# tud-amr/mpc_planner

Hardware: AMD Instinct MI355X
Metric: MPC solves/s (Jackal N=20, 8 obs) (higher is better)
Workload: dtype f64

## Files before the change

mpc_planner_amd/csrc/tmpc_kernels.hpp:

```cpp
#pragma once
#include <hip/hip_runtime.h>
#include <math.h>
#include <stdint.h>
#include <stdio.h>
#include <stdlib.h>
#include <string.h>
#include <string>
#include <type_traits>
#include <vector>

#include "../../include/tmpc_hip.h"
#include "tmpc_stage.hpp"

namespace tmpc {

constexpr int NT = 64;

static __constant__ int c_pi[NP28] = {0, 1, 1, 2, 2, 2, 3, 3, 3, 3, 4, 4, 4, 4, 4, 5, 5, 5, 5, 5, 5, 6, 6, 6, 6, 6, 6, 6};
static __constant__ int c_pj[NP28] = {0, 0, 1, 0, 1, 2, 0, 1, 2, 3, 0, 1, 2, 3, 4, 0, 1, 2, 3, 4, 5, 0, 1, 2, 3, 4, 5, 6};

enum { ST_KEEP_ITERATE = 1, ST_KEEP_MULTIPLIERS = 2, ST_STORE = 4, ST_COMPLETE = 8 };
struct StateIO {
    double *z;
    double *pi;
    double *lamh;
    int *stopped;
    int flags;
    double *ws;
    int *ticket;
    const int *slot;
    int *valid;
    const int *share;
};
__device__ __forceinline__ int param_base_of(const StateIO &io, int b) { return io.share ? io.share[b] : b; }
__device__ __forceinline__ int slot_of(const StateIO &io, int b) { return io.slot ? io.slot[b] : b; }
__device__ __forceinline__ int slot_flags(const StateIO &io, int b)
{
    if (!(io.flags & (ST_KEEP_ITERATE | ST_KEEP_MULTIPLIERS))) return io.flags;
    return io.valid[slot_of(io, b)] ? io.flags : (io.flags & ~(ST_KEEP_ITERATE | ST_KEEP_MULTIPLIERS));
}

struct Lds {
    double *z, *pi, *W, *g, *BA, *b, *D, *beta;
    double *t, *lam, *invt, *qt;
    double *v, *pq, *Hh, *rg, *gh, *rb, *dv, *dpi, *pr, *y, *rdiag, *scr;
    double *dyn8;
    double *lamh;
    int nh, NG, GB, XB, nrows;
    double *tab;
    int n_pair, dstride;
    double *scan;
};

constexpr int BAC_1 = 8, BAC_SDT = 9, BAC_SH = 10, BAC_0 = 11, BAC_DT = 12, BA_NCONST = 20;
constexpr int BAR_S = 5, BAR_PSI = 12, BAR_V = 13;
constexpr int BAP_X = 16, BAP_Y = 15, BAP_S = 7;
constexpr int BAT_A = 3, BAT_W = 6, BAT_XY = 7, BAT_PSI = 16, BAT_V = 9, BAT_S = 17;
constexpr unsigned ba_pack(int a, int w, int x, int y, int p, int v, int s_)
{
    return (unsigned)a | (unsigned)w << 4 | (unsigned)x << 8 | (unsigned)y << 12 | (unsigned)p << 16 | (unsigned)v << 20 | (unsigned)s_ << 24;
}
__device__ __forceinline__ constexpr unsigned ba_rowcode(int m)
{
    return m == 0 ? ba_pack(0, 2, BAC_1, BAC_0, 4, 6, BAC_0)
         : m == 1 ? ba_pack(1, 3, BAC_0, BAC_1, 5, 7, BAC_0)
         : m == 2 ? ba_pack(BAC_0, BAC_DT, BAC_0, BAC_0, BAC_1, BAC_0, BAC_0)
         : m == 3 ? ba_pack(BAC_DT, BAC_0, BAC_0, BAC_0, BAC_0, BAC_1, BAC_0)
                  : ba_pack(BAC_SH, BAC_0, BAC_0, BAC_0, BAC_0, BAC_SDT, BAC_1);
}
__device__ __forceinline__ int ba_off(int N, int k, int m, int j)
{
    const unsigned rc = m == 0 ? ba_rowcode(0) : m == 1 ? ba_rowcode(1) : m == 2 ? ba_rowcode(2) : m == 3 ? ba_rowcode(3) : ba_rowcode(4);
    const int code = (int)((rc >> (4 * j)) & 15u);
    return code < 8 ? k * 8 + code : N * 8 + code - 8;
}
__device__ __forceinline__ void ba_tab_init(double *tab, const Dims &d, int tid)
{
    if (tid < BA_NCONST) {
        const double dt = d.dt, sdt = d.sdt, sh = d.shdt2;
        const double c[BA_NCONST] = {1.0, sdt, sh, 0.0, dt,   sh, dt, 0.0, 0.0, 0.0, 1.0, sdt,   0.0, dt, dt, 0.0, 1.0, 0.0, 0.0, 1.0};
        double val = 0.0;
#pragma unroll
        for (int i = 0; i < BA_NCONST; i++) if (i == tid) val = c[i];
        tab[d.N * 8 + tid] = val;
    }
}
__host__ __device__ inline int ws_doubles(int N, bool two_wave = false)
{
    return (N + 1) * NV + (N + 1) * NX + (N + 1) * NP28 + (N + 1) * NV + (N + 1) * NX + (two_wave ? N * NP28 : 0);
}


__host__ __device__ inline int lds_doubles(int N, int nh)
{
    const int nrows = N * nh + 4 * N + 10 * (N - 1);
    int n = 0;
    n += (N + 1) * NV + (N + 1) * NX + (N + 1) * NP28 + (N + 1) * NV + N * NX * NV + N * NX + N * nh * 3 + N * nh;
    n += 4 * nrows;
    n += (N + 1) * NV + (N + 1) * NX + (N + 1) * NP28 + 2 * (N + 1) * NV + N * NX + (N + 1) * NV + (N + 1) * NX +
         (N + 1) * NX + N * NU + N * NU + 64 + N * 8;
    return n;
}

__host__ __device__ inline bool split_rows_for(int N, int nh)
{
    return 2 * N * nh <= (N + 1) * (NV + NX + NP28 + NV + NV) + N * NX && 12 * (N + 1) >= 12 * N;
}

__device__ __forceinline__ Lds carve(double *s, const Dims &d)
{
    Lds L;
    const int N = d.N;
    L.nh = d.n_up + d.M;
    L.NG = N * L.nh; L.GB = L.NG; L.XB = L.NG + 4 * N; L.nrows = L.XB + 10 * (N - 1);
    auto take = [&](int n) { double *p = s; s += n; return p; };
    L.z = take((N + 1) * NV); L.pi = take((N + 1) * NX); L.W = take((N + 1) * NP28); L.g = take((N + 1) * NV);
    L.BA = take(N * NX * NV); L.b = take(N * NX); L.D = take(N * L.nh * 3); L.beta = take(N * L.nh);
    L.t = take(L.nrows); L.lam = take(L.nrows); L.invt = take(L.nrows); L.qt = take(L.nrows);
    L.v = take((N + 1) * NV); L.pq = take((N + 1) * NX); L.Hh = take((N + 1) * NP28);
    L.rg = take((N + 1) * NV); L.gh = take((N + 1) * NV); L.rb = take(N * NX); L.dv = take((N + 1) * NV);
    L.dpi = take((N + 1) * NX); L.pr = take((N + 1) * NX); L.y = take(N * NU); L.rdiag = take(N * NU);
    L.scr = take(64); L.dyn8 = take(N * 8);
    L.lamh = nullptr;
    return L;
}

__device__ __forceinline__ int trajectory_of_block(int blk, int B)
{
    (void)B;
    return blk;
}

template <int CTRL, int ROW_MASK>
__device__ __forceinline__ double dpp_move(double x, double identity)
{
    union { double d; int i[2]; } u, o;
    u.d = x; o.d = identity;
    o.i[0] = __builtin_amdgcn_update_dpp(o.i[0], u.i[0], CTRL, ROW_MASK, 0xf, false);
    o.i[1] = __builtin_amdgcn_update_dpp(o.i[1], u.i[1], CTRL, ROW_MASK, 0xf, false);
    return o.d;
}
template <int CTRL>
__device__ __forceinline__ double dpp_shift_zero(double x)
{
    union { double d; int i[2]; } u, o;
    u.d = x;
    o.i[0] = __builtin_amdgcn_mov_dpp(u.i[0], CTRL, 0xf, 0xf, true);
    o.i[1] = __builtin_amdgcn_mov_dpp(u.i[1], CTRL, 0xf, 0xf, true);
    return o.d;
}
template <typename Op>
__device__ __forceinline__ double wave_reduce(double x, double identity, Op op)
{
    x = op(x, dpp_move<0x111, 0xf>(x, identity));
    x = op(x, dpp_move<0x112, 0xf>(x, identity));
    x = op(x, dpp_move<0x114, 0xf>(x, identity));
    x = op(x, dpp_move<0x118, 0xf>(x, identity));
    x = op(x, dpp_move<0x142, 0xa>(x, identity));
    x = op(x, dpp_move<0x143, 0xc>(x, identity));
    union { double d; int i[2]; } u;
    u.d = x;
    u.i[0] = __builtin_amdgcn_readlane(u.i[0], 63);
    u.i[1] = __builtin_amdgcn_readlane(u.i[1], 63);
    return u.d;
}
__device__ __forceinline__ double wave_max(double x)
{
    return wave_reduce(x, -__builtin_huge_val(), [](double a, double b) { return fmax(a, b); });
}
__device__ __forceinline__ double wave_min(double x)
{
    return wave_reduce(x, __builtin_huge_val(), [](double a, double b) { return fmin(a, b); });
}
__device__ __forceinline__ double wave_sum(double x)
{
    return wave_reduce(x, 0.0, [](double a, double b) { return a + b; });
}

template <int NTH, typename Op>
__device__ __forceinline__ double blk_combine(double x, double *scr, int tid, int slot, Op op)
{
    if constexpr (NTH == 64) return x;
    constexpr int NW = NTH / 64;
    if ((tid & 63) == 0) scr[slot * NW + (tid >> 6)] = x;
    __syncthreads();
    double r = scr[slot * NW];
#pragma unroll
    for (int w = 1; w < NW; w++) r = op(r, scr[slot * NW + w]);
    return r;
}
template <int NTH> __device__ __forceinline__ double blk_max(double x, double *scr, int tid, int slot = 0)
{
    return blk_combine<NTH>(wave_max(x), scr, tid, slot, [](double a, double b) { return fmax(a, b); });
}
template <int NTH> __device__ __forceinline__ double blk_min(double x, double *scr, int tid, int slot = 0)
{
    return blk_combine<NTH>(wave_min(x), scr, tid, slot, [](double a, double b) { return fmin(a, b); });
}
template <int NTH> __device__ __forceinline__ double blk_sum(double x, double *scr, int tid, int slot = 0)
{
    return blk_combine<NTH>(wave_sum(x), scr, tid, slot, [](double a, double b) { return a + b; });
}

template <int NTH>
__device__ __forceinline__ void blk_residuals(double &worst, double g, double b, double dd, double m, double &mu, double *scr, int tid)
{
    worst = wave_max(fmax(fmax(g, b), fmax(dd, m))); mu = wave_sum(mu);
    if constexpr (NTH > 64) {
        constexpr int NW = NTH / 64;
        if ((tid & 63) == 0) { const int w = tid >> 6; scr[w] = worst; scr[NW + w] = mu; }
        __syncthreads();
        double v[2 * NW];
#pragma unroll
        for (int i = 0; i < 2 * NW; i++) v[i] = scr[i];
        worst = v[0]; mu = v[NW];
#pragma unroll
        for (int w = 1; w < NW; w++) { worst = fmax(worst, v[w]); mu = mu + v[NW + w]; }
    }
}

struct Row { int k, var, general; double sgn; };

__device__ __forceinline__ Row row_decode(const Lds &L, const Dims &d, int r)
{
    Row R;
    if (r < L.NG) {
        R.k = r / L.nh; const int j = r - R.k * L.nh;
        R.general = r; R.var = -1; R.sgn = (j < d.n_up) ? -1.0 : 1.0;
    } else if (r < L.XB) {
        const int q = r - L.GB;
        R.k = q >> 2; R.var = (q >> 1) & 1; R.general = -1; R.sgn = (q & 1) ? -1.0 : 1.0;
    } else {
        const int q = r - L.XB;
        R.k = 1 + q / 10; const int rem = q - (R.k - 1) * 10;
        R.var = 2 + (rem >> 1); R.general = -1; R.sgn = (rem & 1) ? -1.0 : 1.0;
    }
    return R;
}
__device__ __forceinline__ double row_dot(const Lds &L, const Row &R, const double *vec)
{
    const double *vk = vec + R.k * NV;
    if (R.general >= 0) {
        const double *Dr = L.D + R.general * 3;
        return Dr[0] * vk[ZX] + Dr[1] * vk[ZY] + Dr[2] * vk[ZPSI];
    }
    return vk[R.var];
}
__device__ __forceinline__ double row_beta(const Lds &L, const Dims &d, const Row &R)
{
    if (R.general >= 0) return L.beta[R.general];
    return (R.sgn > 0.0 ? d.lb[R.var] : d.ub[R.var]) - L.z[R.k * NV + R.var];
}

__device__ __forceinline__ double readlane_d(double x, int src)
{
    union { double d; int i[2]; } u;
    u.d = x;
    u.i[0] = __builtin_amdgcn_readlane(u.i[0], src);
    u.i[1] = __builtin_amdgcn_readlane(u.i[1], src);
    return u.d;
}
template <int LANE>
__device__ __forceinline__ double bcast16(double x)
{
    static_assert(LANE >= 0 && LANE < 16, "row_newbcast lane");
    const long long r = __builtin_amdgcn_mov_dpp(__builtin_bit_cast(long long, x), 0x150 + LANE, 0xf, 0xf, false);
    return __builtin_bit_cast(double, r);
}
template <int A, int B, typename F>
__device__ __forceinline__ void static_for(F &&f)
{
    if constexpr (A < B) { f(std::integral_constant<int, A>{}); static_for<A + 1, B>(f); }
}
__device__ __forceinline__ int mul24(int a, int b) { return (int)__umul24((unsigned)a, (unsigned)b); }
__device__ __forceinline__ int uni(int x) { asm volatile("" : "+s"(x)); return x; }
__device__ __forceinline__ double rsqrt_nr(double d)
{
    const double y = __builtin_amdgcn_rsq(d);
    const double e = fma(-d * y, y, 1.0);
    return fma(y, e * fma(0.375, e, 0.5), y);
}

}
#include "tmpc_riccati.hpp"
namespace tmpc {

__device__ void build_rhs(const Lds &L, const Dims &d, int tid, bool predictor)
{
    const int N = d.N;
    for (int it = tid; it < (N + 1) * NV; it += NT) {
        const int k = it / NV, i = it - k * NV;
        double acc = L.rg[it];
        if (i < NU) {
            if (k < N) {
                for (int side = 0; side < 2; side++) {
                    const int r = L.GB + k * 4 + i * 2 + side;
                    const double sgn = side ? -1.0 : 1.0;
                    const double beta = (side ? d.ub[i] : d.lb[i]) - L.z[k * NV + i];
                    const double rd = sgn * (L.v[k * NV + i] - beta) - L.t[r];
                    const double q = predictor ? L.lam[r] : L.qt[r];
                    acc += sgn * (q + L.lam[r] * L.invt[r] * rd);
                }
            }
        } else if (k >= 1 && k < N) {
            for (int side = 0; side < 2; side++) {
                const int r = L.XB + (k - 1) * 10 + (i - NU) * 2 + side;
                const double sgn = side ? -1.0 : 1.0;
                const double beta = (side ? d.ub[i] : d.lb[i]) - L.z[k * NV + i];
                const double rd = sgn * (L.v[k * NV + i] - beta) - L.t[r];
                const double q = predictor ? L.lam[r] : L.qt[r];
                acc += sgn * (q + L.lam[r] * L.invt[r] * rd);
            }
        }
        if (k < N && i >= ZX && i <= ZPSI) {
            const double *vk = L.v + k * NV;
            for (int j = 0; j < L.nh; j++) {
                const int r = k * L.nh + j;
                const double sgn = (j < d.n_up) ? -1.0 : 1.0;
                const double *Dr = L.D + r * 3;
                const double cv = Dr[0] * vk[ZX] + Dr[1] * vk[ZY] + Dr[2] * vk[ZPSI];
                const double rd = sgn * (cv - L.beta[r]) - L.t[r];
                const double q = predictor ? L.lam[r] : L.qt[r];
                acc += sgn * Dr[i - ZX] * (q + L.lam[r] * L.invt[r] * rd);
            }
        }
        L.gh[it] = acc;
    }
    __syncthreads();
}

enum { PH_LIN = 0, PH_RES, PH_HH, PH_FACTOR, PH_RHS, PH_SOLVE, PH_ROWS, PH_UPDATE, PH_FINAL, PH_TOTAL, PH_COUNT };
struct Prof {
    long long *out; long long acc[PH_COUNT]; long long t0;
    __device__ __forceinline__ void init(long long *o) { out = o; for (int i = 0; i < PH_COUNT; i++) acc[i] = 0; }
    __device__ __forceinline__ void start() { if (out) t0 = clock64(); }
    __device__ __forceinline__ void stop(int ph) { if (out) { const long long t1 = clock64(); acc[ph] += t1 - t0; t0 = t1; } }
    __device__ __forceinline__ void finish(int tid, int b, long long t_begin)
    {
        if (!out) return;
        stop(PH_FINAL);
        acc[PH_TOTAL] = clock64() - t_begin;
        if (tid == 0) for (int i = 0; i < PH_COUNT; i++) out[(size_t)b * PH_COUNT + i] = acc[i];
    }
};
struct NoProf {
    __device__ __forceinline__ void init(long long *) {}
    __device__ __forceinline__ void start() {}
    __device__ __forceinline__ void stop(int) {}
    __device__ __forceinline__ void finish(int, int, long long) {}
};

__device__ int ipm_solve(const Lds &L, const Dims &d, int tid, int *iters_out, Prof &pf)
{
    const int N = d.N;
    const double m_rows = (double)L.nrows;
    for (int r = tid; r < L.nrows; r += NT) {
        const Row R = row_decode(L, d, r);
        const double rr = R.sgn * (row_dot(L, R, L.v) - row_beta(L, d, R));
        const double t = rr > d.thr0 ? rr : d.thr0;
        L.t[r] = t; L.invt[r] = 1.0 / t; L.lam[r] = d.mu0 / t;
    }
    __syncthreads();
    int status = 2, iters = 0;
    for (int it = 0;; it++) {
        pf.start();
        double res_g = 0.0, res_b = 0.0, res_d = 0.0, res_m = 0.0, mu = 0.0;
        for (int e = tid; e < (N + 1) * NV; e += NT) {
            const int k = e / NV, i = e - k * NV;
            double acc = 0.0;
            const bool skip = (k == N && i < NU) || (k == 0 && i >= NU);
            if (!skip) {
                acc = L.g[e];
                const double *Wk = L.W + k * NP28; const double *vk = L.v + k * NV;
#pragma unroll
                for (int j = 0; j < NV; j++) acc += Wk[sidx(i, j)] * vk[j];
                if (k < N) {
                    const double *BA = L.BA + k * NX * NV;
#pragma unroll
                    for (int l = 0; l < NX; l++) acc += BA[l * NV + i] * L.pq[(k + 1) * NX + l];
                }
                if (i >= NU && k >= 1) acc -= L.pq[k * NX + i - NU];
                if (i < NU) {
                    const int r = L.GB + k * 4 + i * 2;
// ... 687 lines not shown
```

mpc_planner_amd/csrc/tmpc_riccati.hpp:

```cpp
#pragma once

namespace tmpc {

#ifdef TMPC_SWEEP_PROFILE
enum { SP_FACTOR_TERM = 0, SP_FACTOR_LOOP, SP_SOLVE_PRE, SP_SOLVE_BWD, SP_SOLVE_FWD, SP_SOLVE_POST, SP_CALLS_FACTOR, SP_CALLS_SOLVE, SP_COUNT };
__device__ unsigned long long g_sweep_prof[SP_COUNT];
#define SWEEP_T0(lead) long long sp_t = clock64(); const bool sp_lead = (lead)
#define SWEEP_T(i) do { const long long sp_n = clock64(); if (sp_lead) atomicAdd(&g_sweep_prof[i], (unsigned long long)(sp_n - sp_t)); sp_t = sp_n; } while (0)
#define SWEEP_COUNT(i) do { if (tid == 0) atomicAdd(&g_sweep_prof[i], 1ull); } while (0)
#else
#define SWEEP_T0(lead)
#define SWEEP_T(i)
#define SWEEP_COUNT(i)
#endif

#if defined(__HIP_DEVICE_COMPILE__)
#define TMPC_PRIO_HIGH() do { if (d.prio) __builtin_amdgcn_s_setprio(3); } while (0)
#define TMPC_PRIO_LOW() do { if (d.prio) __builtin_amdgcn_s_setprio(2); } while (0)
#define TMPC_PRIO_LINEARISE() do { if (d.prio) __builtin_amdgcn_s_setprio(0); } while (0)
#else
#define TMPC_PRIO_HIGH()
#define TMPC_PRIO_LOW()
#define TMPC_PRIO_LINEARISE()
#endif
// ... 100 lines not shown
        } else {
            const double *Hk = L.Hh + hoff<CP>(k);
#pragma unroll
            for (int j = 0; j < NV; j++) o.hk[j] = Hk[pidx(ls, j <= ls ? j : ls)];
            if constexpr (CP) {
                { const double *Tc = L.tab + bc.o0 + mul24(k, bc.st); o.ba[0] = Tc[0]; o.ba[1] = Tc[1]; }
#pragma unroll
                for (int m = 2; m < NX; m++) o.ba[m] = bac[m];
            } else {
                const double *BA = L.BA + k * NX * NV;
#pragma unroll
                for (int m = 0; m < NX; m++) o.ba[m] = BA[m * NV + ls];
            }
        }
    };
#pragma unroll
    for (int j = 0; j < NV; j++) f[j] = (j >= NU) ? (vec ? L.gh[N * NV + j] : L.Hh[hoff<CP>(N) + pidx(ls, j <= ls ? j : ls)]) : 0.0;
    Opnd oa, ob;
    load_stage(oa, N - 1);
    if constexpr (SQ) bad |= chol_rows<NU>(f, li, nullptr, nullptr);
    const bool prl = rowl && li >= NU, vl = vec && wr;
    const int dum = (int)(L.scr - L.Hh) + (CP ? RDUM_BASE_COMPACT : RDUM_BASE_FULL);
    const int po = vl ? (int)(L.pr - L.Hh) : prl ? FB_P + i5 * (i5 + 1) / 2 : dum + RDUM_P, pst = vl ? NX : prl ? hstride<CP>() : 0;
    const int qo = vl ? (CP == 3 ? NP28 : (int)(L.y - L.Hh)) : prl ? FB_LXU + 2 * i5 : dum + RDUM_PAIR;
    const int qst = vl ? (CP == 3 ? hstride<CP>() : NU) : prl ? hstride<CP>() : 0;
    const int vo = (rowl && li == 1) ? 0 : dum + RDUM_PIV - FB_R0, vst = (rowl && li == 1) ? hstride<CP>() : 0;
    auto store_pairs = [&](int k, double r0, double r1) {
        double *pp = L.Hh + qo + mul24(k, qst);
        pp[0] = f[0]; pp[1] = f[1];
        double *Fv = L.Hh + vo + mul24(k, vst);
        Fv[FB_L10] = f[0]; Fv[FB_R0] = r0; Fv[FB_R1] = r1;
    };
    auto stage = [&](const Opnd &o, Opnd &nx, int k) {
        double Pm[NX][NX];
        static_for<0, NX>([&](auto m_) {
            constexpr int m = decltype(m_)::value;
#pragma unroll
            for (int l = 0; l <= m; l++) Pm[m][l] = bcast16<NU + m>(f[NU + l]);
        });
        {
            double *Ln = L.Hh + po + mul24(k + 1, pst);
            Ln[4] = f[NU + 4]; Ln[3] = f[NU + 3];
            asm volatile("" ::: "memory");
            Ln[2] = f[NU + 2];
            asm volatile("" ::: "memory");
            Ln[1] = f[NU + 1];
            asm volatile("" ::: "memory");
            Ln[0] = f[NU + 0];
        }
        if constexpr (SQ) {
            double Go[NX];
#pragma unroll
            for (int l = 0; l < NX; l++) {
                double acc = 0.0;
#pragma unroll
                for (int m = l; m < NX; m++) acc += Pm[m][l] * o.ba[m];
                Go[l] = VEC ? fma(vmask, f[NU + l], acc) : acc;
            }
            const double Xa = bcast16<ZA>(o.ba[0]), Ya = bcast16<ZA>(o.ba[1]), Xw = bcast16<ZW>(o.ba[0]), Yw = bcast16<ZW>(o.ba[1]);
            const double Xp = bcast16<ZPSI>(o.ba[0]), Yp = bcast16<ZPSI>(o.ba[1]), Xv = bcast16<ZV>(o.ba[0]), Yv = bcast16<ZV>(o.ba[1]);
            double Ga[NX], Gw[NX], Gp[3], Gv[NX];
            Ga[0] = ((Pm[0][0] * Xa + Pm[1][0] * Ya) + Pm[3][0] * dt) + Pm[4][0] * shdt2;
            Ga[1] = (Pm[1][1] * Ya + Pm[3][1] * dt) + Pm[4][1] * shdt2;
            Ga[2] = Pm[3][2] * dt + Pm[4][2] * shdt2;
            Ga[3] = Pm[3][3] * dt + Pm[4][3] * shdt2;
            Ga[4] = Pm[4][4] * shdt2;
            Gw[0] = (Pm[0][0] * Xw + Pm[1][0] * Yw) + Pm[2][0] * dt;
            Gw[1] = Pm[1][1] * Yw + Pm[2][1] * dt;
            Gw[2] = Pm[2][2] * dt; Gw[3] = 0.0; Gw[4] = 0.0;
            Gp[0] = (Pm[0][0] * Xp + Pm[1][0] * Yp) + Pm[2][0];
            Gp[1] = Pm[1][1] * Yp + Pm[2][1];
            Gp[2] = Pm[2][2];
            Gv[0] = ((Pm[0][0] * Xv + Pm[1][0] * Yv) + Pm[3][0]) + Pm[4][0] * sdt;
            Gv[1] = (Pm[1][1] * Yv + Pm[3][1]) + Pm[4][1] * sdt;
            Gv[2] = Pm[3][2] + Pm[4][2] * sdt;
            Gv[3] = Pm[3][3] + Pm[4][3] * sdt;
            Gv[4] = Pm[4][4] * sdt;
            double a0 = o.hk[ZA], a1 = o.hk[ZW], a2 = o.hk[ZX], a3 = o.hk[ZY], a4 = o.hk[ZPSI], a5 = o.hk[ZV], a6 = o.hk[ZS];
#pragma unroll
            for (int l = 0; l < NX; l++) {
                a0 += Go[l] * Ga[l];
                if (l < 3) a1 += Go[l] * Gw[l];
                if (l < 1) a2 += Go[l] * Pm[0][0];
                if (l < 2) a3 += Go[l] * Pm[1][l];
                if (l < 3) a4 += Go[l] * Gp[l];
                a5 += Go[l] * Gv[l];
                a6 += Go[l] * Pm[4][l];
            }
            f[ZA] = a0; f[ZW] = a1; f[ZX] = a2; f[ZY] = a3; f[ZPSI] = a4; f[ZV] = a5; f[ZS] = a6;
            load_stage(nx, k > 0 ? k - 1 : 0);
            double r0 = 0.0, r1 = 0.0;
            bad |= chol_rows<0>(f, li, &r0, &r1);
            store_pairs(k, r0, r1);
            return;
        }
        double w[NX];
#pragma unroll
        for (int n = 0; n < NX; n++) {
            double acc = Pm[n > 0 ? n : 0][0] * o.ba[0];
#pragma unroll
            for (int m = 1; m < NX; m++) acc = fma(Pm[m > n ? m : n][m > n ? n : m], o.ba[m], acc);
            w[n] = VEC ? fma(vmask, f[NU + n], acc) : acc;
        }
        {
            const double Xa = bcast16<ZA>(o.ba[0]), Ya = bcast16<ZA>(o.ba[1]), Xw = bcast16<ZW>(o.ba[0]), Yw = bcast16<ZW>(o.ba[1]);
            const double Xp = bcast16<ZPSI>(o.ba[0]), Yp = bcast16<ZPSI>(o.ba[1]), Xv = bcast16<ZV>(o.ba[0]), Yv = bcast16<ZV>(o.ba[1]);
            f[ZA] = fma(w[4], shdt2, fma(w[3], dt, fma(w[1], Ya, fma(w[0], Xa, o.hk[ZA]))));
            f[ZW] = fma(w[2], dt, fma(w[1], Yw, fma(w[0], Xw, o.hk[ZW])));
            f[ZX] = o.hk[ZX] + w[0];
            f[ZY] = o.hk[ZY] + w[1];
            f[ZPSI] = fma(w[1], Yp, fma(w[0], Xp, o.hk[ZPSI])) + w[2];
            f[ZV] = fma(w[4], sdt, fma(w[1], Yv, fma(w[0], Xv, o.hk[ZV])) + w[3]);
            f[ZS] = o.hk[ZS] + w[4];
        }
        load_stage(nx, k > 0 ? k - 1 : 0);
        double r0 = 0.0, r1 = 0.0;
        bad |= chol_rows<0, NU>(f, li, &r0, &r1);
        store_pairs(k, r0, r1);
    };
    if constexpr (CP == 0) {
        int k = N - 1;
        for (; k >= 1; k -= 2) {
            stage(oa, ob, k);
            stage(ob, oa, k - 1);
        }
        if (k == 0) stage(oa, ob, 0);
    } else {
        for (int k = N - 1; k >= 0; k--) stage(oa, oa, k);
    }
    return bad;
}

template <int NTH, int CP = 0, bool VEC = false, bool SQ = false>
__device__ __forceinline__ bool riccati_factor(const Lds &L, const Dims &d, int tid, int sw = 0)
{
    asm volatile("" : "+v"(tid));
    bool anybad = false;
    SWEEP_T0(tid == 0); SWEEP_COUNT(SP_CALLS_FACTOR);
    if (NTH == 64 || (tid >> 6) == sw) {
        const int lane = tid & 63;
        TMPC_PRIO_HIGH();
        const bool bad = riccati_factor_rows<CP, VEC, SQ>(L, d, lane, true);
        TMPC_PRIO_LOW();
        bool bad_p = false;
        if constexpr (!SQ) {
            const unsigned *Pd = reinterpret_cast<const unsigned *>(L.Hh + hoff_lane<CP>(lane < d.N ? lane + 1 : d.N) + FB_P) + 1;
            bad_p = (int)(Pd[2 * 0] | Pd[2 * 2] | Pd[2 * 5] | Pd[2 * 9] | Pd[2 * 14]) < 0;
        }
        anybad = __any((bad && lane < 16) || bad_p);
        if (NTH > 64 && lane == 0) L.scr[63] = anybad ? 1.0 : 0.0;
    }
    __syncthreads();
    SWEEP_T(SP_FACTOR_LOOP);
    if (NTH > 64) anybad = L.scr[63] != 0.0;
    return anybad;
}

template <int CP, bool SQ = false>
__device__ __forceinline__ void riccati_solve_pre(const Lds &L, const Dims &d, int tid, int nth)
{
    const int N = d.N;
    for (int k = tid; k < N; k += nth) {
        const double *Pn = L.Hh + hoff_lane<CP>(k + 1) + FB_P;
        const double *r = L.rb + mul24(k, NX);
        double pp[15], rr[NX];
#pragma unroll
        for (int e = 0; e < 15; e++) pp[e] = Pn[e];
#pragma unroll
        for (int m = 0; m < NX; m++) rr[m] = r[m];
        if constexpr (SQ) {
            double tl[NX];
#pragma unroll
            for (int l = 0; l < NX; l++) {
                double acc = 0.0;
#pragma unroll
                for (int m = l; m < NX; m++) acc += pp[m * (m + 1) / 2 + l] * rr[m];
                tl[l] = acc;
            }
#pragma unroll
            for (int i = 0; i < NX; i++) {
                double acc = 0.0;
#pragma unroll
                for (int l = 0; l <= i; l++) acc += pp[i * (i + 1) / 2 + l] * tl[l];
                L.dpi[mul24(k + 1, NX) + i] = acc;
            }
            continue;
        }
#pragma unroll
        for (int i = 0; i < NX; i++) {
            double acc = 0.0;
#pragma unroll
            for (int m = 0; m < NX; m++) acc += pp[(m > i ? m * (m + 1) / 2 + i : i * (i + 1) / 2 + m)] * rr[m];
            L.dpi[mul24(k + 1, NX) + i] = acc;
        }
    }
}
template <int CP, bool SQ = false>
__device__ __forceinline__ void riccati_solve_post(const Lds &L, const Dims &d, int tid, int nth)
{
    const int N = d.N;
    for (int kk = tid; kk < N; kk += nth) {
        const int k = kk + 1;
        const double *Pk = L.Hh + hoff_lane<CP>(k) + FB_P;
        const double *dxk = L.dv + mul24(k, NV) + NU;
        double pp[15], rr[NX], pk[NX];
#pragma unroll
        for (int e = 0; e < 15; e++) pp[e] = Pk[e];
#pragma unroll
        for (int m = 0; m < NX; m++) { rr[m] = dxk[m]; pk[m] = L.pr[mul24(k, NX) + m]; }
        if constexpr (SQ) {
            double tl[NX];
#pragma unroll
            for (int l = 0; l < NX; l++) {
                double acc = 0.0;
#pragma unroll
                for (int m = l; m < NX; m++) acc += pp[m * (m + 1) / 2 + l] * rr[m];
                tl[l] = acc;
            }
#pragma unroll
            for (int i = 0; i < NX; i++) {
                double acc = 0.0;
#pragma unroll
                for (int l = 0; l <= i; l++) acc += pp[i * (i + 1) / 2 + l] * tl[l];
                L.dpi[mul24(k, NX) + i] = acc + pk[i];
            }
            continue;
        }
#pragma unroll
        for (int i = 0; i < NX; i++) {
            double acc = 0.0;
#pragma unroll
            for (int m = 0; m < NX; m++) acc += pp[(m > i ? m * (m + 1) / 2 + i : i * (i + 1) / 2 + m)] * rr[m];
            L.dpi[mul24(k, NX) + i] = acc + pk[i];
        }
    }
}

template <int CP, bool BWD = true, typename MID>
__device__ __forceinline__ void riccati_sweeps_rows(const Lds &L, const Dims &d, int li, bool wr, bool sweeper, MID mid)
{
    const int N = d.N;
    const bool rowl = li < NV && wr, xl = rowl && li >= NU;
    const int ls = li < NV ? li : 0;
    const int i5 = (li >= NU && li < NV) ? li - NU : 0;
    SWEEP_T0(li == 0);
    if constexpr (BWD) {
    if (sweeper) {
    double p = L.gh[N * NV + ls];
    {
        struct Ops { double ghj, ba[NX], a0, a1; };
        const int fbo = li < NU ? FB_R0 + li : FB_LXU + 2 * i5;
        const BaLane bc = ba_column(N, ls);
        double bac[NX];
        if constexpr (CP) {
#pragma unroll
            for (int m = 2; m < NX; m++) bac[m] = L.tab[ba_off(N, 0, m, ls)];
        }
        const bool ql = li >= 8 && li < 8 + NX;
        const double *ghq = ql ? L.dpi + NX + (li - 8) : L.gh + ls;
        const int ghs = ql ? NX : NV;
        auto load_stage = [&](Ops &o, int k) {
            const double *Fb = L.Hh + hoff<CP>(k);
            o.ghj = ghq[mul24(k, ghs)];
            if constexpr (CP) {
                { const double *Tc = L.tab + bc.o0 + mul24(k, bc.st); o.ba[0] = Tc[0]; o.ba[1] = Tc[1]; }
#pragma unroll
                for (int l = 2; l < NX; l++) o.ba[l] = bac[l];
            } else {
                const double *BA = L.BA + k * NX * NV;
#pragma unroll
                for (int l = 0; l < NX; l++) o.ba[l] = BA[l * NV + ls];
            }
            o.a0 = Fb[fbo]; o.a1 = Fb[fbo + 1];
        };
        auto stage = [&](const Ops &o, int k) {
            const double Pb = p + dpp_shift_zero<0x106>(o.ghj);
            double fj = o.ghj;
            static_for<0, NX>([&](auto l_) { constexpr int l = decltype(l_)::value; fj += o.ba[l] * bcast16<NU + l>(Pb); });
            const double y0 = bcast16<0>(fj * o.a0);
            const double y1 = bcast16<1>((fj - o.a0 * y0) * o.a1);
            p = fj - o.a0 * y0 - o.a1 * y1;
            if (rowl && li == 0) { ysl<CP>(L, k)[0] = y0; ysl<CP>(L, k)[1] = y1; }
            if (xl) L.pr[k * NX + i5] = p;
        };
        Ops oa, ob;
        load_stage(oa, N - 1);
        if (xl) L.pr[N * NX + i5] = p;
        int k = N - 1;
        for (; k >= 1; k -= 2) {
            load_stage(ob, k - 1);
            stage(oa, k);
            load_stage(oa, k >= 2 ? k - 2 : 0);
            stage(ob, k - 1);
        }
        if (k == 0) stage(oa, 0);
    }
    }
    mid();
    }
    SWEEP_T(SP_SOLVE_BWD);
    if (sweeper) {
        double dx = 0.0;
        struct Ops { double yr, a0, a1, a_psi, a_v, b_a, b_w; };
        const double *yrb = li < NU ? ysl<CP>(L, 0) + li : L.rb + i5;
        const int yrs = li < NU ? (CP == 3 ? hstride<CP>() : NU) : NX;
        const int fbo = li < NU ? FB_R0 + li : FB_LXU + 2 * i5;
        const double i_psi = li == ZPSI ? 1.0 : 0.0, i_v = li == ZV ? 1.0 : 0.0;
        double *dv_own = L.dv + ls;
        const BaLane br = ba_row4(N, i5);
        auto load_stage = [&](Ops &o, int k) {
            const double *Fb = L.Hh + hoff<CP>(k);
            o.yr = yrb[mul24(k, yrs)];
            o.a0 = Fb[fbo]; o.a1 = Fb[fbo + 1];
            if constexpr (CP) {
                const double *Tr = L.tab + br.o0 + mul24(k, br.st);
                o.a_psi = Tr[4]; o.a_v = Tr[6];
                o.b_a = Tr[0]; o.b_w = Tr[2];
            } else {
                const double *BAr = L.BA + k * NX * NV + i5 * NV;
                o.a_psi = BAr[ZPSI]; o.a_v = BAr[ZV];
                o.b_a = BAr[ZA]; o.b_w = BAr[ZW];
            }
        };
        auto stage = [&](const Ops &o, int k) {
            const double p0 = o.a0 * dx, p1 = o.a1 * dx;
            double s0 = o.yr, s1 = o.yr;
            static_for<0, NX>([&](auto m_) { constexpr int m = decltype(m_)::value; s0 += bcast16<NU + m>(p0); s1 += bcast16<NU + m>(p1); });
            double dxs[NX];
            dxs[ZPSI - NU] = bcast16<ZPSI>(dx); dxs[ZV - NU] = bcast16<ZV>(dx);
            const double u1 = bcast16<1>(-s1 * o.a1);
            const double u0 = bcast16<0>((-s0 - o.a1 * u1) * o.a0);
            if (rowl && li == 0) { L.dv[k * NV] = u0; L.dv[k * NV + 1] = u1; }
            if (xl) dv_own[k * NV] = dx;
            const double dpsi = dxs[ZPSI - NU], dvv = dxs[ZV - NU];
            const double e_psi = o.a_psi - i_psi, e_v = o.a_v - i_v;
            dx = dx + e_psi * dpsi + e_v * dvv + o.b_a * u0 + o.b_w * u1 + o.yr;
        };
        Ops oa, ob;
        load_stage(oa, 0);
        int k = 0;
        for (; k + 1 < N; k += 2) {
            load_stage(ob, k + 1);
            stage(oa, k);
            load_stage(oa, k + 2 < N ? k + 2 : N - 1);
            stage(ob, k + 1);
        }
        if (k < N) stage(oa, k);
        if (rowl) L.dv[N * NV + li] = xl ? dx : 0.0;
    }
    SWEEP_T(SP_SOLVE_FWD);
}

template <int NTH, int CP = 0, bool SQ = false>
__device__ __forceinline__ void riccati_solve(const Lds &L, const Dims &d, int tid, int sw = 1)
{
    asm volatile("" : "+v"(tid));
    const bool sweeper = NTH == 64 || (tid >> 6) == sw;
    const int lane = NTH == 64 ? tid : (sweeper ? (tid & 63) : 64);
    SWEEP_COUNT(SP_CALLS_SOLVE);
    riccati_solve_pre<CP, SQ>(L, d, tid, NTH);
    __syncthreads();
    TMPC_PRIO_HIGH();
    riccati_sweeps_rows<CP, true>(L, d, lane, true, sweeper, [] { __syncthreads(); });
    TMPC_PRIO_LOW();
    __syncthreads();
    riccati_solve_post<CP, SQ>(L, d, tid, NTH);
    __syncthreads();
}

template <int NTH, int CP = 0>
__device__ __forceinline__ void riccati_forward(const Lds &L, const Dims &d, int tid, int sw = 1)
{
    asm volatile("" : "+v"(tid));
    const bool sweeper = NTH == 64 || (tid >> 6) == sw;
    const int lane = NTH == 64 ? tid : (sweeper ? (tid & 63) : 64);
    SWEEP_COUNT(SP_CALLS_SOLVE);
    TMPC_PRIO_HIGH();
    riccati_sweeps_rows<CP, false>(L, d, lane, true, sweeper, [] {});
    TMPC_PRIO_LOW();
    __syncthreads();
}

}
```

Before: 1.562 million.

## Split forward Riccati sweep across two lane groups and reorder BA constant table

The forward substitution sweep now maps the second control row onto a separate group of lanes (lanes 8..), so each lane computes a single accumulation with one DPP shift per state instead of two broadcast reductions per lane. The constant table layout is permuted and folded so the identity subtraction is baked in for the compact path, which removes per-stage subtractions. The aim is to shorten the serial dependency chain of each forward stage, at the cost of a more intricate lane mapping and new constant-offset assumptions that must stay consistent with the table.

After: 1.603 million (median of 6 runs). 2.6% higher.

```diff
diff --git a/mpc_planner_amd/csrc/tmpc_kernels.hpp b/mpc_planner_amd/csrc/tmpc_kernels.hpp
--- a/mpc_planner_amd/csrc/tmpc_kernels.hpp
+++ b/mpc_planner_amd/csrc/tmpc_kernels.hpp
@@ -52,10 +52,10 @@
     double *scan;
 };
 
-constexpr int BAC_1 = 8, BAC_SDT = 9, BAC_SH = 10, BAC_0 = 11, BAC_DT = 12, BA_NCONST = 20;
-constexpr int BAR_S = 5, BAR_PSI = 12, BAR_V = 13;
-constexpr int BAP_X = 16, BAP_Y = 15, BAP_S = 7;
-constexpr int BAT_A = 3, BAT_W = 6, BAT_XY = 7, BAT_PSI = 16, BAT_V = 9, BAT_S = 17;
+constexpr int BAC_SH = 8, BAC_DT = 9, BAC_0 = 10, BAC_1 = 13, BAC_SDT = 14, BA_NCONST = 20;
+constexpr int BAR_S = 0, BAR_PSI = 8, BAR_V = 11;
+constexpr int BAP_X = 7, BAP_Y = 4, BAP_S = 2;
+constexpr int BAT_A = 17, BAT_W = 1, BAT_XY = 2, BAT_PSI = 7, BAT_V = 4, BAT_S = 3;
 constexpr unsigned ba_pack(int a, int w, int x, int y, int p, int v, int s_)
 {
     return (unsigned)a | (unsigned)w << 4 | (unsigned)x << 8 | (unsigned)y << 12 | (unsigned)p << 16 | (unsigned)v << 20 | (unsigned)s_ << 24;
@@ -78,7 +78,7 @@
 {
     if (tid < BA_NCONST) {
         const double dt = d.dt, sdt = d.sdt, sh = d.shdt2;
-        const double c[BA_NCONST] = {1.0, sdt, sh, 0.0, dt,   sh, dt, 0.0, 0.0, 0.0, 1.0, sdt,   0.0, dt, dt, 0.0, 1.0, 0.0, 0.0, 1.0};
+        const double c[BA_NCONST] = {sh, dt, 0.0, 0.0, 0.0, 1.0, sdt,   1.0, 0.0, 0.0, dt, dt, 0.0, 0.0, 0.0, 0.0, 0.0,   0.0, dt, sh};
         double val = 0.0;
 #pragma unroll
         for (int i = 0; i < BA_NCONST; i++) if (i == tid) val = c[i];
diff --git a/mpc_planner_amd/csrc/tmpc_riccati.hpp b/mpc_planner_amd/csrc/tmpc_riccati.hpp
--- a/mpc_planner_amd/csrc/tmpc_riccati.hpp
+++ b/mpc_planner_amd/csrc/tmpc_riccati.hpp
@@ -426,12 +426,14 @@
     if (sweeper) {
         double dx = 0.0;
         struct Ops { double yr, a0, a1, a_psi, a_v, b_a, b_w; };
-        const double *yrb = li < NU ? ysl<CP>(L, 0) + li : L.rb + i5;
-        const int yrs = li < NU ? (CP == 3 ? hstride<CP>() : NU) : NX;
-        const int fbo = li < NU ? FB_R0 + li : FB_LXU + 2 * i5;
-        const double i_psi = li == ZPSI ? 1.0 : 0.0, i_v = li == ZV ? 1.0 : 0.0;
+        const bool shb = li >= 8 && li < 8 + NV;
+        const int lj = shb ? li - 8 : ls, j5 = lj >= NU ? lj - NU : 0;
+        const double *yrb = lj < NU ? ysl<CP>(L, 0) + (shb ? 1 : 0) : L.rb + j5;
+        const int yrs = lj < NU ? (CP == 3 ? hstride<CP>() : NU) : NX;
+        const int fbo = lj < NU ? (shb ? FB_R1 : FB_R0) : FB_LXU + 2 * j5 + (shb ? 1 : 0);
+        const double i_psi = lj == ZPSI ? 1.0 : 0.0, i_v = lj == ZV ? 1.0 : 0.0;
         double *dv_own = L.dv + ls;
-        const BaLane br = ba_row4(N, i5);
+        const BaLane br = ba_row4(N, j5);
         auto load_stage = [&](Ops &o, int k) {
             const double *Fb = L.Hh + hoff<CP>(k);
             o.yr = yrb[mul24(k, yrs)];
@@ -441,23 +443,23 @@
                 o.a_psi = Tr[4]; o.a_v = Tr[6];
                 o.b_a = Tr[0]; o.b_w = Tr[2];
             } else {
-                const double *BAr = L.BA + k * NX * NV + i5 * NV;
+                const double *BAr = L.BA + k * NX * NV + j5 * NV;
                 o.a_psi = BAr[ZPSI]; o.a_v = BAr[ZV];
                 o.b_a = BAr[ZA]; o.b_w = BAr[ZW];
             }
         };
         auto stage = [&](const Ops &o, int k) {
-            const double p0 = o.a0 * dx, p1 = o.a1 * dx;
-            double s0 = o.yr, s1 = o.yr;
-            static_for<0, NX>([&](auto m_) { constexpr int m = decltype(m_)::value; s0 += bcast16<NU + m>(p0); s1 += bcast16<NU + m>(p1); });
+            const double pa = o.a0 * dx;
+            double s = o.yr;
+            static_for<0, NX>([&](auto m_) { constexpr int m = decltype(m_)::value; s += dpp_shift_zero<0x100 + NU + m>(pa); });
             double dxs[NX];
             dxs[ZPSI - NU] = bcast16<ZPSI>(dx); dxs[ZV - NU] = bcast16<ZV>(dx);
-            const double u1 = bcast16<1>(-s1 * o.a1);
-            const double u0 = bcast16<0>((-s0 - o.a1 * u1) * o.a0);
+            const double u1 = bcast16<8>(-s * o.a0);
+            const double u0 = bcast16<0>((-s - o.a1 * u1) * o.a0);
             if (rowl && li == 0) { L.dv[k * NV] = u0; L.dv[k * NV + 1] = u1; }
             if (xl) dv_own[k * NV] = dx;
             const double dpsi = dxs[ZPSI - NU], dvv = dxs[ZV - NU];
-            const double e_psi = o.a_psi - i_psi, e_v = o.a_v - i_v;
+            const double e_psi = CP ? o.a_psi : o.a_psi - i_psi, e_v = CP ? o.a_v : o.a_v - i_v;
             dx = dx + e_psi * dpsi + e_v * dvv + o.b_a * u0 + o.b_w * u1 + o.yr;
         };
         Ops oa, ob;
```
